# ScanNet/ScanNet

Measured on AMD Instinct MI355X. Metric: RGB-D frames/sec integrated (640x480, 4 mm voxel), higher is better.
Workload: dtype f32; 1 GPU; configs[1]: scene0000_00-scale synthetic stream (5578-frame box-room walk, 640x480 u16 depth, 4 mm voxels, 2^19 hash buckets x 10, 2^20 SDF blocks), frames 5..24 per rank, depth AND colour (a 640x480 RGB8 frame per depth frame, 921 600 B) resident in HBM; frames_per_pass=32, blocks_live_end=34141, alloc_failures=0

## Files before the change

include/scanfuse_internal.h:

```cpp
#ifndef SCANFUSE_INTERNAL_H
#define SCANFUSE_INTERNAL_H

#include "scanfuse.h"

#ifdef __cplusplus
extern "C" {
#endif

int sf_fuser_tune(sf_fuser* f, const char* key, int value);

int sf_fuser_alloc_probe_count(sf_fuser* f, uint64_t* out);

int sf_fuser_alloc_direct_count(sf_fuser* f, uint64_t* out);

int sf_fuser_mc_timing(const sf_fuser* f, double* out, int n);

int sf_zlib_inflate_gpu(const void* src, uint64_t src_bytes, uint64_t expect_bytes, int device, void* dst);
int sf_zlib_inflate_gpu_bench(const void* const* srcs, const uint64_t* src_bytes, int count, uint64_t expect_bytes, int device, int repeats, int skip, double* us_tokens, double* us_copy);

int sf_fuse_run_device_counts(uint64_t out[4]);

int sf_jpeg_decode_gpu_huffman(const uint8_t* data, uint64_t bytes, uint32_t width, uint32_t height, int device, uint8_t* dst_rgb);

int sf_fuser_profile_enable(sf_fuser* f, int on);
// ... 2 lines not shown
int sf_synth_room_device(void* d_depth, uint64_t frame_stride_bytes, uint64_t first_frame, uint64_t n, uint64_t total_frames,
                         int width, int height, int noise, float* poses_out);
int sf_synth_scan_device(void* d_depth, uint64_t frame_stride_bytes, uint64_t first_frame, uint64_t n, uint64_t total_frames,
                         int width, int height, int noise, const double room_m[3], const double origin_m[3], float* poses_out);

int sf_synth_scene_device(void* d_depth, uint64_t frame_stride_bytes, uint64_t first_frame, uint64_t n, uint64_t total_frames,
                          int width, int height, int noise, int scene, uint32_t seed, const double room_m[3], const double origin_m[3],
                          float* poses_out);
int sf_synth_clutter_boxes(const double room_m[3], uint32_t seed, float* lo_out , float* hi_out , int* n_out);

struct sf_mesh;
int sf_simplify_probe_edge(const struct sf_mesh* in, const sf_simplify_params* p, uint32_t v0, uint32_t v1, double quadric10[10], float position[3],
                           float* priority, double* scale_factor);

int sf_simplify_stage_edges(int device, uint32_t V, uint32_t F, const float* pos, const uint32_t* tri, const uint8_t* alive, const double* Q_in ,
                            const sf_simplify_params* p, double scale, uint64_t needed, int stalled, uint32_t* E_out, uint64_t* ukey, uint32_t* ucnt,
                            double* Q_out, float* pri, float* x, float* tau_out, double* scale_out );
int sf_simplify_stage_winners(int device, uint32_t V, uint32_t F, const uint32_t* tri, const uint8_t* alive, uint32_t E_in, const float* pri, float tau,
                              uint32_t round, uint8_t* pass_out, uint8_t* taken_out, uint32_t counters[3]);
int sf_simplify_stage_collapse(int device, uint32_t V, uint32_t F, float* pos, uint32_t* tri, uint8_t* alive, double* Q, uint32_t n, const uint32_t* edges,
                               uint32_t E_in, const float* x, uint8_t* vdel_out);

int sf_clean_stage_merge(int device, uint32_t V, const float* pos, float radius, uint32_t* target_out, uint32_t* launches_out, uint32_t* cells_out,
                         uint32_t* merged_out);
int sf_clean_stage_faces(int device, uint32_t V, uint32_t F, const uint32_t* tri, const uint32_t* target , uint8_t* verdict_out, uint32_t* tri_out,
                         uint32_t* degenerate_out, uint32_t* duplicate_out);
int sf_clean_stage_components(int device, uint32_t F, const uint32_t* tri, uint32_t min_faces, uint32_t* root_out, uint32_t* size_out, uint8_t* keep_out,
                              uint32_t counters[3]);
int sf_clean_stage_compact(int device, uint32_t V, uint32_t F, const float* pos, const uint8_t* col , const uint32_t* tri, uint32_t* used_out,
                           uint32_t* remap_out, float* pos_out, uint8_t* col_out, uint32_t* tri_out, uint32_t* vertices_out);
int sf_clean_probe_merge(uint32_t V, const float* pos, float radius, uint32_t* target_out);

int sf_selftest_division(int device, uint64_t* recip_mismatches, uint64_t* quot_mismatches, uint64_t* div_mismatches);

int sf_fuser_calib_tile_rmw(sf_fuser* f, int read_only, int iters, double* avg_us, uint32_t* tiles);
int sf_fuser_calib_tile_rmw_ex(sf_fuser* f, int mode, int iters, double* avg_us, uint32_t* tiles);

int sf_fuser_track_system(sf_fuser* f, const uint16_t* depth, int level, const float T[16], const float T_ref[16], const sf_track_params* t,
                          double sys[29], uint8_t* mask);

int sf_fuser_track_rgbd_system(sf_fuser* f, const uint16_t* depth, const uint8_t* rgb, int level, const float T[16], const float T_ref[16],
                               const sf_track_params* t, double sys[31], uint8_t* mask);

int sf_fuser_align_system(sf_fuser* f, const uint16_t* depth, uint64_t K, const float* poses, const int32_t* pairs, uint64_t P, const sf_align_params* a,
                          double* sys);
int sf_fuser_align_rgbd_system(sf_fuser* f, const uint16_t* depth, const uint8_t* rgb, uint64_t K, const float* poses, const int32_t* pairs, uint64_t P,
                               const sf_align_params* a, double* sys);

int sf_align_group_solve_stage(int device, uint64_t G, const int32_t* group_first, const int32_t* pair_first, const int32_t* local_pairs,
                               const uint32_t* valid_masks, const double* sys, int nsys, int min_pair_correspondences, double* xi_out, int32_t* status_out,
                               int32_t* used_out, uint32_t* conn_out, double* sums_out);

int sf_filter2d_stage_prepare(int device, const uint16_t* depth16, int dn, const uint8_t* rgb, int cn, float* depth_out, float* intensity_out);
int sf_filter2d_stage_bilateral(int device, const float* in, float sigma_d, float sigma_r, int w, int h, float* out);
int sf_filter2d_stage_resample_float(int device, const float* in, int iw, int ih, float* out, int ow, int oh);
int sf_filter2d_stage_resample_uchar(int device, const uint8_t* in, int iw, int ih, uint8_t* out, int ow, int oh);
int sf_filter2d_stage_vote(int device, const uint8_t* instance_in, const float* depth, const float* intensity, const uint8_t instance_to_idx[256],
                           const uint8_t idx_to_instance[80], int radius, int w, int h, float sigma_d, float sigma_r, float intensity_scale,
                           uint8_t* instance_out);
int sf_filter2d_stage_to_label(int device, const uint8_t* instance, const uint16_t instance_to_label[256], int n, uint16_t* label_out);
int sf_filter2d_selftest_gauss(int device, float sigma, const float* dist, const int32_t* dx, const int32_t* dy, uint64_t n, float* out_r, float* out_d);

int sf_axis_align_stage_up(const struct sf_sens* sens, uint32_t gravity_min_records, float up3[3], int32_t* source, uint64_t* no_gravity);
int sf_axis_align_stage_normals(const float* xyz, uint64_t num_vertices, const uint32_t* tris, uint64_t num_faces, int device, float* normals_out);
int sf_axis_align_stage_planes(const float* xyz, const float* normals, uint64_t num_vertices, const sf_axis_align_params* p, int device, uint32_t* index_out,
                               uint64_t* n_founded, uint32_t* ids, float* table10, uint32_t* counts, uint32_t* behind, uint64_t capacity, uint64_t* n_sorted,
// ... 31 lines not shown
```

scannet_amd/csrc/calib.hip:

```cpp
#include <hip/hip_runtime.h>

#include "common.h"
#include "fuser_internal.h"

namespace {
__global__ __launch_bounds__(256) void k_calib_rmw(uint4* __restrict__ buf, size_t n16) {
  for (size_t i = (size_t)blockIdx.x * 256 + threadIdx.x; i < n16; i += (size_t)gridDim.x * 256) {
    uint4 v = buf[i];
    v.x += 1u; v.y ^= v.x; v.z += v.y; v.w ^= v.z;
    buf[i] = v;
  }
}
__global__ __launch_bounds__(256) void k_calib_read(const uint4* __restrict__ buf, size_t n16, uint32_t* sink) {
  uint32_t acc = 0;
  for (size_t i = (size_t)blockIdx.x * 256 + threadIdx.x; i < n16; i += (size_t)gridDim.x * 256) {
    const uint4 v = buf[i];
    acc ^= v.x ^ v.y ^ v.z ^ v.w;
  }
  if (acc == 0x12345u) *sink = acc;
}
}

SF_API int sf_calib_stream(int device, uint64_t bytes, int iters) {
  SF_HIP_CHECK(hipSetDevice(device));
// ... 34 lines not shown
    const uint32_t e = 100u + (uint32_t)(x >> 58);
    n0 = __uint_as_float(((uint32_t)x & 0x807FFFFFu) | (e << 23));
    const float qf = __uint_as_float(0x3F800000u | ((uint32_t)(x >> 24) & 0x7FFFFFu));
    n1 = __uint_as_float(__float_as_uint(qf * m) + ((uint32_t)(x >> 50) & 7u) - 3u);
  }
  const v2f q = quot_rn((v2f){n0, n1}, splat(m), splat(r));
  unsigned int n = (__float_as_uint(q.x) != __float_as_uint(n0 / m)) + (__float_as_uint(q.y) != __float_as_uint(n1 / m));
  if (n) atomicAdd(bad, (unsigned long long)n);
}
__global__ __launch_bounds__(256) void k_selftest_div(unsigned long long* bad) {
  const uint64_t i = (uint64_t)blockIdx.x * 256 + threadIdx.x;
  uint64_t x = (i + 1) * 0x9E3779B97F4A7C15ull;
  x ^= x >> 29; x *= 0xBF58476D1CE4E5B9ull; x ^= x >> 32;
  uint64_t y = (x ^ 0xD6E8FEB86659FD93ull) * 0x94D049BB133111EBull;
  y ^= y >> 31;
  const uint32_t eb = 103u + (uint32_t)(x >> 58) % 41u;
  const uint32_t ea = 97u + (uint32_t)(y >> 58) % 43u;
  const float b = __uint_as_float(((uint32_t)x & 0x807FFFFFu) | (eb << 23));
  const float a0 = __uint_as_float(((uint32_t)y & 0x807FFFFFu) | (ea << 23));
  const float qf = __uint_as_float(0x3F800000u | ((uint32_t)(y >> 24) & 0x7FFFFFu));
  const float a1 = __uint_as_float(__float_as_uint(qf * b) + ((uint32_t)(x >> 50) & 7u) - 3u);
  const float qh = __uint_as_float(__float_as_uint(qf) & 0xFFFFFFFEu);
  const float a2 = __uint_as_float(__float_as_uint(fmaf(qh, b, 0x1p-24f * b)) + ((uint32_t)(y >> 50) & 7u) - 3u);
  const float a3 = __uint_as_float(__float_as_uint(a0) ^ 0x00400000u);
  const float rb = recip_rn(b);
  unsigned int n = 0;
  n += __float_as_uint(div_rn(a0, b, rb)) != __float_as_uint(a0 / b);
  n += __float_as_uint(div_rn(a1, b, rb)) != __float_as_uint(a1 / b);
  n += __float_as_uint(div_rn(a2, b, rb)) != __float_as_uint(a2 / b);
  n += __float_as_uint(div_rn(a3, b, rb)) != __float_as_uint(a3 / b);
  n += __float_as_uint(rb) != __float_as_uint(1.0f / b);
  if (n) atomicAdd(bad, (unsigned long long)n);
}
}

SF_API int sf_selftest_division(int device, uint64_t* recip_mismatches, uint64_t* quot_mismatches, uint64_t* div_mismatches) {
  if (!recip_mismatches || !quot_mismatches || !div_mismatches) return sf::fail(SF_ERR_INVALID_ARG, "NULL argument");
  SF_HIP_CHECK(hipSetDevice(device));
  unsigned long long* d = nullptr;
  SF_HIP_CHECK(hipMalloc((void**)&d, 24));
  SF_HIP_CHECK(hipMemset(d, 0, 24));
  hipLaunchKernelGGL(k_selftest_recip, dim3((1u << 23) / 256), dim3(256), 0, nullptr, d);
  hipLaunchKernelGGL(k_selftest_quot, dim3((1u << 20) / 256, 511), dim3(256), 0, nullptr, d + 1);
  hipLaunchKernelGGL(k_selftest_div, dim3((1u << 26) / 256), dim3(256), 0, nullptr, d + 2);
  unsigned long long h[3] = {0, 0, 0};
  const hipError_t e = hipMemcpy(h, d, 24, hipMemcpyDeviceToHost);
  (void)hipFree(d);
  if (e != hipSuccess) return sf::fail(SF_ERR_DEVICE, "self-test failed: %s", hipGetErrorString(e));
  *recip_mismatches = h[0];
  *quot_mismatches = h[1];
  *div_mismatches = h[2];
  return SF_OK;
}
```

scannet_amd/csrc/fuser_alloc.hip:

```cpp
#include <hip/hip_runtime.h>

#include <algorithm>
#include <climits>
#include <cmath>

#include "fuser_device.h"
#include "fuser_internal.h"

namespace {

__device__ inline int world_to_block(float w, float voxel, float rv) {
  const float q = div_rn(w, voxel, rv);
  const int vi = (int)(q >= 0.0f ? q + 0.5f : q - 0.5f);
  return vi >> 3;
}

constexpr int ALLOC_SET = 256;
constexpr int ALLOC_LIST = 512;
constexpr int ALLOC_SET_PROBES = 32;

template <int WIN_LOG2, bool MULTI>
__global__ __launch_bounds__(256) void k_alloc(const float* __restrict__ depthf_all, HashEntry* table, int32_t* heap,
                                               uint64_t* block_keys, int32_t* block_entry, uint8_t* block_flags, int32_t* counters, ParamsK P,
                                               BatchFrames B, int group_frames, BrickCache bricks) {
// ... 444 lines not shown
    const float slu = du_ * inv * (float)sgn, slv = dv_ * inv * (float)sgn;
    const float a0 = ((float)k0 + 0.5f) - oa;
    const float iu = ou_ + du_ * inv * a0 - (float)(RW_LAT / 2), iv = ov_ + dv_ * inv * a0 - (float)(RW_LAT / 2);
    const float fiu = floorf(iu), fiv = floorf(iv);
    w_axis = __builtin_amdgcn_readfirstlane(axis); w_k0 = __builtin_amdgcn_readfirstlane(k0); w_sgn = __builtin_amdgcn_readfirstlane(sgn);
    w_su = __builtin_amdgcn_readfirstlane((int)rintf(slu * 4096.0f)); w_ou = __builtin_amdgcn_readfirstlane((int)fiu);
    w_fu = __builtin_amdgcn_readfirstlane((int)((iu - fiu) * 4096.0f));
    w_sv = __builtin_amdgcn_readfirstlane((int)rintf(slv * 4096.0f)); w_ov = __builtin_amdgcn_readfirstlane((int)fiv);
    w_fv = __builtin_amdgcn_readfirstlane((int)((iv - fiv) * 4096.0f));
  };
  int n_map = max(1, j_end - j_begin);
  if (MULTI && j_end - j_begin > 1) {
    float d0[3], o0[3], d1[3], o1[3];
    centre_ray(j_begin, d0, o0);
    centre_ray(j_end - 1, d1, o1);
    const float far = P.maxd / bs;
    float D = 0.0f;
#pragma unroll
    for (int r = 0; r < 3; r++) D = fmaxf(D, fabsf((o1[r] + d1[r] * far) - (o0[r] + d0[r] * far)));
    if (D > 9.0f) n_map = max(1, (int)((float)(j_end - j_begin) * 9.0f / D));
    n_map = __builtin_amdgcn_readfirstlane(n_map);
  }
  int next_map = j_begin;
  const bool in_image = x < P.W && y < P.H;
  const float kx = ((float)x - P.mx) / P.fx, ky = ((float)y - P.my) / P.fy;
  const float rvoxel = 1.0f / P.voxel;
  float d_next;
  if (fuse_depth16 != nullptr) {
    if (blockIdx.x == 0 && blockIdx.y == 0 && threadIdx.x == 0) atomicExch(reinterpret_cast<unsigned long long*>(&counters[compact_counter]), 0ull);
    d_next = -INFINITY;
    if (in_image) {
      const uint16_t u = fuse_depth16[(size_t)(y * P.W + x)];
      float v = (float)u / P.depth_shift;
      if (u == 0 || v < P.dmin || v > P.dmax) v = -INFINITY;
      depthf_out[(size_t)(y * P.W + x)] = v;
      d_next = v;
    }
  } else {
    d_next = in_image && j_begin < j_end ? depthf_all[(size_t)j_begin * npx + (size_t)(y * P.W + x)] : -INFINITY;
  }
  __syncthreads();
  for (int j = j_begin; j < j_end; ++j) {
    const FrameK& F = B.f[j];
    const float d_cur = d_next;
    d_next = in_image && j + 1 < j_end ? depthf_all[(size_t)(j + 1) * npx + (size_t)(y * P.W + x)] : -INFINITY;
    if (j == next_map) {
      anchor(j, min(j + n_map, j_end) - 1);
      next_map = j + n_map;
      if (MULTI && j != j_begin)
        for (int i = threadIdx.x; i < RW_WORDS / 4; i += 256) s_done4[i] = make_uint4(0, 0, 0, 0);
    }

    bool active = false;
    int a_cx = 0, a_cy = 0, a_cz = 0, a_sx = 0, a_sy = 0, a_sz = 0, a_ex = 0, a_ey = 0, a_ez = 0;
    float a_tmx = INFINITY, a_tmy = INFINITY, a_tmz = INFINITY, a_tdx = INFINITY, a_tdy = INFINITY, a_tdz = INFINITY;
    if (in_image) {
      const float d = d_cur;
      if (d != -INFINITY && d < P.maxd) {
        const float t = fmaf(P.tscale, d, P.tbase);
        const float lo = min_f32(P.maxd, d - t);
        const float hi = min_f32(P.maxd, d + t);
        if (lo < hi) {
          float p0[3], p1[3];
          {
            const float ax = kx * lo, ay = ky * lo, az = lo;
#pragma unroll
            for (int r = 0; r < 3; r++) p0[r] = fmaf(F.T[4 * r], ax, fmaf(F.T[4 * r + 1], ay, fmaf(F.T[4 * r + 2], az, F.T[4 * r + 3])));
// ... 211 lines not shown
```

scannet_amd/csrc/fuser_fuse.h:

```cpp
#pragma once
#include <hip/hip_runtime.h>

#include "fuser_device.h"
#include "fuser_internal.h"

namespace {


constexpr int RTAB = 512;

struct FrameV {
  float ti[12];
  float fx, fy, mx, my, tscale, tbase;
};
__device__ inline FrameV frame_constants(const ParamsK& P, const float* __restrict__ Ti) {
  FrameV F;
#pragma unroll
  for (int k = 0; k < 12; k++) F.ti[k] = Ti[k];
  F.fx = P.fx; F.fy = P.fy; F.mx = P.mx; F.my = P.my;
  F.tscale = P.tscale; F.tbase = P.tbase;
  return F;
}

__device__ inline int cvt_i32(float x) {
  int r;
  asm("v_cvt_i32_f32 %0, %1" : "=v"(r) : "v"(x));
  return r;
}

__device__ inline uint32_t add_sat_u32(uint32_t a, uint32_t b) {
  uint32_t r;
  asm("v_add_u32_e64 %0, %1, %2 clamp" : "=v"(r) : "v"(a), "s"(b));
  return r;
}

__device__ inline int depth_weight(const ParamsK& P, float d) {
  const float z01 = (d - P.dmin) / (P.dmax - P.dmin);
  const float wf = fmaxf(((float)P.wsample * 1.5f) * (1.0f - z01), 1.0f);
  return min(cvt_i32(wf), 255);
}

template <int J0, int NJ, bool CLAMP>
__device__ inline void fuse_project(const ParamsK& P, const FrameV& FV, v2f wx, float wy, const float (&wz)[4], v2f (&pz)[NJ],
                                    uint32_t (&pix)[2 * NJ], bool (&ok)[2 * NJ]) {
  const float* Ti = FV.ti;
  const uint32_t uw = (uint32_t)P.W, uh = (uint32_t)P.H;
  v2f axy[NJ], azz[NJ / 2];
#pragma unroll
  for (int j = 0; j < NJ; j++)
    axy[j] = pk_fma((v2f){Ti[1], Ti[5]}, splat(wy), pk_fma((v2f){Ti[2], Ti[6]}, splat(wz[J0 + j]), (v2f){Ti[3], Ti[7]}));
#pragma unroll
  for (int jj = 0; jj < NJ / 2; jj++)
    azz[jj] = pk_fma(splat(Ti[9]), splat(wy), pk_fma(splat(Ti[10]), (v2f){wz[J0 + 2 * jj], wz[J0 + 2 * jj + 1]}, splat(Ti[11])));
#pragma unroll
  for (int j = 0; j < NJ; j++) {
    const v2f pcx = pk_fma(splat(Ti[0]), wx, splat(axy[j].x));
    const v2f pcy = pk_fma(splat(Ti[4]), wx, splat(axy[j].y));
    const v2f pcz = pk_fma(splat(Ti[8]), wx, splat(azz[j >> 1][j & 1]));
    const v2f rz = recip_rn(pcz);
    const v2f uf = pk_add(pk_fma(pcx * splat(FV.fx), rz, splat(FV.mx)), splat(0.5f));
    const v2f vf = pk_add(pk_fma(pcy * splat(FV.fy), rz, splat(FV.my)), splat(0.5f));
    pz[j] = pcz;
#pragma unroll
    for (int hx = 0; hx < 2; hx++) {
      const uint32_t px = (uint32_t)cvt_i32(uf[hx]), py = (uint32_t)cvt_i32(vf[hx]);
      const bool in = (pcz[hx] > 0.0f) && (px < uw) && (py < uh);
      const uint32_t p = __umul24(py, uw) + px;
      ok[2 * j + hx] = in;
      pix[2 * j + hx] = CLAMP ? (in ? p : 0u) : p;
    }
  }
}

template <int J0, int NJ>
__device__ inline void fuse_project_xr(const ParamsK& P, const FrameV& FV, const v2f (&wxp)[4], float wy, float wz, v2f (&pz)[NJ],
                                       uint32_t (&pix)[2 * NJ], bool (&ok)[2 * NJ]) {
  const float* Ti = FV.ti;
  const uint32_t uw = (uint32_t)P.W, uh = (uint32_t)P.H;
  const float ax = fmaf(Ti[1], wy, fmaf(Ti[2], wz, Ti[3]));
  const float ay = fmaf(Ti[5], wy, fmaf(Ti[6], wz, Ti[7]));
  const float az = fmaf(Ti[9], wy, fmaf(Ti[10], wz, Ti[11]));
#pragma unroll
  for (int j = 0; j < NJ; j++) {
    const v2f pcx = pk_fma(splat(Ti[0]), wxp[J0 + j], splat(ax));
    const v2f pcy = pk_fma(splat(Ti[4]), wxp[J0 + j], splat(ay));
    const v2f pcz = pk_fma(splat(Ti[8]), wxp[J0 + j], splat(az));
    const v2f rz = recip_rn(pcz);
    const v2f uf = pk_add(pk_fma(pcx * splat(FV.fx), rz, splat(FV.mx)), splat(0.5f));
    const v2f vf = pk_add(pk_fma(pcy * splat(FV.fy), rz, splat(FV.my)), splat(0.5f));
    pz[j] = pcz;
#pragma unroll
    for (int hx = 0; hx < 2; hx++) {
      const uint32_t px = (uint32_t)cvt_i32(uf[hx]), py = (uint32_t)cvt_i32(vf[hx]);
      const bool in = (pcz[hx] > 0.0f) && (px < uw) && (py < uh);
      ok[2 * j + hx] = in;
      pix[2 * j + hx] = __umul24(py, uw) + px;
    }
  }
}

template <int SIGN, int COLOR, bool TAB, int WM, int J0, int NJ, bool ROWS = true>
__device__ inline void fuse_update(const ParamsK& P, const FrameV& FV, const v2f (&rcp_m)[NJ], const float (&d)[2 * NJ], const uint32_t (&c)[2 * NJ], const v2f (&pz)[NJ],
                                   const bool (&ok)[2 * NJ], uint4 (&v)[4], uint64_t (&dirty)[4]) {
  constexpr bool WS1 = WM == 1 || WM == 2;
  const float wn = (float)P.wsample;
  const uint32_t round_mask = P.colour_round ? 0x010101u : 0u;
  const uint32_t first_mask = P.colour_first ? 0x00FFFFFFu : 0xFF000000u;
  constexpr bool wdep = WM == 3;
  const uint32_t maxd_bits = __float_as_uint(P.maxd);
  v2f q[NJ], sdfc[NJ];
  v2f wnv[NJ];
  int wni[2 * NJ];
  uint32_t ncw[2 * NJ];
  bool upd[2 * NJ];
  bool sat[2 * NJ];
  bool any_upd = false;
#pragma unroll
  for (int j = 0; j < NJ; j++) {
    const v2f dk = {d[2 * j], d[2 * j + 1]};
    v2f sdf = dk - pz[j];
    const v2f t = pk_fma(splat(FV.tscale), dk, splat(FV.tbase));
#pragma unroll
    for (int hx = 0; hx < 2; hx++) {
      upd[2 * j + hx] = ok[2 * j + hx] && (__float_as_uint(dk[hx]) < maxd_bits) && (sdf[hx] > -t[hx]);
      sdf[hx] = min_f32(sdf[hx], t[hx]);
      sat[2 * j + hx] = false;
      any_upd = any_upd || upd[2 * j + hx];
      wni[2 * j + hx] = wdep ? depth_weight(P, dk[hx]) : P.wsample;
    }
    wnv[j] = wdep ? (v2f){(float)wni[2 * j], (float)wni[2 * j + 1]} : splat(wn);
    sdfc[j] = sdf;
  }
  if (!__any((int)any_upd)) return;
  bool slow = false;
#pragma unroll
  for (int j = 0; j < NJ; j++) {
    const v2f sdf = sdfc[j];
    const uint32_t cwj[2] = {v[J0 + j].y, v[J0 + j].w};
    const v2f wo = {(float)(cwj[0] >> 24), (float)(cwj[1] >> 24)};
    const v2f old = {__uint_as_float(v[J0 + j].x), __uint_as_float(v[J0 + j].z)};
    if (SIGN > 0) {
      const v2f n = pk_fma(old, wo, WS1 ? sdf : sdf * wnv[j]);
      const v2f m = wo + wnv[j];
      if (TAB) {
        q[j] = quot_rn(n, m, rcp_m[j]);
        slow = slow || (fabsf(n.x) < 0x1p-100f) || (fabsf(n.y) < 0x1p-100f);
      } else {
        q[j] = (v2f){n.x / m.x, n.y / m.y};
      }
#pragma unroll
      for (int hx = 0; hx < 2; hx++) {
        const uint32_t cw = cwj[hx];
        const uint32_t w = cw >> 24;
        uint32_t rgb = cw;
        if (COLOR) {
          const uint32_t ck = c[2 * j + hx];
          const uint32_t avg = __builtin_amdgcn_lerp(cw, ck, round_mask);
          const bool first = COLOR == 2 ? cw < 0x01000000u : (cw & first_mask) == 0u;
          rgb = first ? ck : avg;
        }
        if (WM == 2) {
          if (COLOR) {
            ncw[2 * j + hx] = (rgb & 0x00FFFFFFu) | (add_sat_u32(cw, 0x01000000u) & 0xFF000000u);
          } else {
            uint32_t inc;
            const bool full = __builtin_add_overflow(cw, 0x01000000u, &inc);
// ... 14 lines not shown
      for (int hx = 0; hx < 2; hx++) {
        const int nw = (int)(cwj[hx] >> 24) - wni[2 * j + hx];
        if (nw <= 0) { q[j][hx] = __uint_as_float(0u); ncw[2 * j + hx] = 0u; }
        else ncw[2 * j + hx] = (cwj[hx] & 0xFFFFFFu) | ((uint32_t)nw << 24);
      }
    }
  }
  if (SIGN > 0 && TAB && __builtin_expect(__any((int)slow), 0)) {
#pragma unroll
    for (int j = 0; j < NJ; j++) {
      const v2f wo = {(float)(v[J0 + j].y >> 24), (float)(v[J0 + j].w >> 24)};
      const v2f old = {__uint_as_float(v[J0 + j].x), __uint_as_float(v[J0 + j].z)};
      const v2f n = pk_fma(old, wo, sdfc[j] * wnv[j]);
      const v2f m = wo + wnv[j];
      q[j] = (v2f){n.x / m.x, n.y / m.y};
    }
  }
#pragma unroll
  for (int j = 0; j < NJ; j++) {
    v[J0 + j].x = upd[2 * j] ? __float_as_uint(q[j].x) : v[J0 + j].x;
    v[J0 + j].y = (upd[2 * j] && !sat[2 * j]) ? ncw[2 * j] : v[J0 + j].y;
    v[J0 + j].z = upd[2 * j + 1] ? __float_as_uint(q[j].y) : v[J0 + j].z;
    v[J0 + j].w = (upd[2 * j + 1] && !sat[2 * j + 1]) ? ncw[2 * j + 1] : v[J0 + j].w;
    if (ROWS) dirty[J0 + j] |= __ballot(upd[2 * j] || upd[2 * j + 1]);
  }
  if (!ROWS) dirty[0] = ~0ull;
}


__device__ inline __amdgpu_buffer_rsrc_t image_rsrc(const void* base, uint32_t bytes) {
  return __builtin_amdgcn_make_buffer_rsrc(const_cast<void*>(base), 0, (int)bytes, 0x00020000);
}

template <int SIGN, int COLOR, bool TAB, int WM, int J0, int NJ, bool ROWS, bool XR = false>
__device__ inline void fuse_rows(const ParamsK& P, const float* __restrict__ Ti, const float* __restrict__ depthf,
                                 const uint2* __restrict__ texel, const float* rtab, v2f wx, float wy, const float (&wz)[4], const v2f (&wxp)[4],
                                 uint4 (&v)[4], uint64_t (&dirty)[4]) {
  v2f pz[NJ], rcp_m[NJ];
  float d[2 * NJ];
  uint32_t c[2 * NJ];
  bool ok[2 * NJ];
  uint32_t pix[2 * NJ];
  if (TAB) {
#pragma unroll
    for (int j = 0; j < NJ; j++) {
      const uint32_t ws = (WM == 1 || WM == 2) ? 1u : (uint32_t)P.wsample;
      rcp_m[j] = (v2f){rtab[(v[J0 + j].y >> 24) + ws], rtab[(v[J0 + j].w >> 24) + ws]};
    }
  }
  const FrameV FV = frame_constants(P, Ti);
  if (XR) fuse_project_xr<J0, NJ>(P, FV, wxp, wy, wz[0], pz, pix, ok);
  else fuse_project<J0, NJ, false>(P, FV, wx, wy, wz, pz, pix, ok);
  const uint32_t img_bytes = (uint32_t)(P.W * P.H) * 4u;
  if (COLOR) {
    typedef uint32_t u32x2 __attribute__((ext_vector_type(2)));
    const __amdgpu_buffer_rsrc_t rt = image_rsrc(texel, 2u * img_bytes);
#pragma unroll
    for (int k = 0; k < 2 * NJ; k++) {
      const u32x2 t = __builtin_amdgcn_raw_buffer_load_b64(rt, pix[k] << 3, 0, 0);
      d[k] = __uint_as_float(t.x);
      c[k] = t.y;
    }
  } else {
    const __amdgpu_buffer_rsrc_t rd = image_rsrc(depthf, img_bytes);
#pragma unroll
    for (int k = 0; k < 2 * NJ; k++) d[k] = __uint_as_float(__builtin_amdgcn_raw_buffer_load_b32(rd, pix[k] << 2, 0, 0));
  }
  fuse_update<SIGN, COLOR, TAB, WM, J0, NJ, ROWS>(P, FV, rcp_m, d, c, pz, ok, v, dirty);
}

}
```

scannet_amd/csrc/fuser_internal.h:

```cpp
#pragma once
#include <hip/hip_runtime.h>

#include <utility>
#include <vector>

#include "common.h"

constexpr uint64_t KEY_EMPTY = ~0ull;
constexpr uint64_t KEY_TOMB = ~0ull - 1ull;
constexpr int MAX_DDA_ITERS = 1024;
constexpr int MAX_PROBES = 4096;
constexpr int MAX_BATCH = 32;
constexpr int DEFAULT_BATCH = 32;

struct HashEntry {
  uint64_t key;
  int32_t ptr;
  uint32_t birth;
};
static_assert(sizeof(HashEntry) == 16, "hash entry is 16 bytes");

struct ParamsK {
  int W, H;
  float fx, fy, mx, my;
// ... 133 lines not shown
    if (t == 0ull) t = tag;
  }
  if (t == tag) atomicOr(e + 1, 1ull << brick_bit(bx, by, bz));
}

#endif

__device__ inline int hash_lookup(const HashEntry* __restrict__ table, const ParamsK& P, int x, int y, int z) {
  const uint64_t key = pack_key(x, y, z);
  uint32_t slot = hash_home(P, x, y, z);
  for (int probe = 0; probe < MAX_PROBES; ++probe) {
    const uint64_t k = table[slot].key;
    if (k == key) return table[slot].ptr;
    if (k == KEY_EMPTY) return -1;
    slot++;
    if (slot == P.total_slots) slot = 0;
  }
  return -1;
}

#ifdef __HIPCC__
struct v2f {
  float x, y;
  __device__ float& operator[](int i) { return i ? y : x; }
  __device__ const float& operator[](int i) const { return i ? y : x; }
};
__device__ inline v2f operator+(v2f a, v2f b) { return v2f{a.x + b.x, a.y + b.y}; }
__device__ inline v2f operator-(v2f a, v2f b) { return v2f{a.x - b.x, a.y - b.y}; }
__device__ inline v2f operator*(v2f a, v2f b) { return v2f{a.x * b.x, a.y * b.y}; }
__device__ inline v2f operator-(v2f a) { return v2f{-a.x, -a.y}; }
__device__ inline v2f pk_fma(v2f a, v2f b, v2f c) { return v2f{__builtin_fmaf(a.x, b.x, c.x), __builtin_fmaf(a.y, b.y, c.y)}; }
__device__ inline v2f splat(float x) { return v2f{x, x}; }
__device__ inline v2f pk_add(v2f a, v2f b) { return a + b; }
__device__ inline v2f recip_rn(v2f b) {
  v2f r = {__builtin_amdgcn_rcpf(b.x), __builtin_amdgcn_rcpf(b.y)};
  const v2f one = splat(1.0f);
  r = pk_fma(pk_fma(-b, r, one), r, r);
  return pk_fma(pk_fma(-b, r, one), r, r);
}
__device__ inline float recip_rn(float b) {
  float r = __builtin_amdgcn_rcpf(b);
  r = fmaf(fmaf(-b, r, 1.0f), r, r);
  return fmaf(fmaf(-b, r, 1.0f), r, r);
}
__device__ inline float div_rn(float a, float b, float y) {
  const float q0 = a * y;
  const float q1 = fmaf(fmaf(-b, q0, a), y, q0);
  return fmaf(fmaf(-b, q1, a), y, q1);
}
__device__ inline v2f quot_rn(v2f n, v2f m, v2f r) {
  const v2f q0 = n * r;
  return pk_fma(pk_fma(-m, q0, n), r, q0);
}
#endif

struct sf_fuser {
  sf_params p;
  ParamsK pk;
  int in_W = 0, in_H = 0;
  size_t in_px = 0;
  int device = 0;
  hipStream_t stream = nullptr;
  hipStream_t front = nullptr;
  hipStream_t front_lo = nullptr;
  hipStream_t last_front = nullptr;
  hipEvent_t ev_front_switch = nullptr;
  int front_prio = -1;
  bool front_lo_lowest = true;
  hipEvent_t ev_compact[2] = {nullptr, nullptr};
  hipEvent_t ev_fused[2] = {nullptr, nullptr};
  hipEvent_t ev_input = nullptr;
  int slot = 0;
  bool serial_tail = false;
// ... 83 lines not shown
```

scannet_amd/csrc/fuser_prepass.hip:

```cpp
#include <hip/hip_runtime.h>

#include <algorithm>
#include <cmath>

#include "fuser_internal.h"
#include "jpeg_idct.h"

namespace {

struct YccPicture {
  int ncomp, sx[3], sy[3], cw[3], ch[3], bw[3];
  const uint8_t* plane[3];
  __device__ YccPicture(const SfJpegLayout* __restrict__ L, const uint8_t* planes) {
    const int W = L->width, H = L->height;
    ncomp = L->ncomp;
    const uint8_t* q = planes;
    for (int c = 0; c < 3; c++) {
      const int cc = c < ncomp ? c : 0;
      sx[c] = L->hmax > L->h[cc] ? 2 : 1; sy[c] = L->vmax > L->v[cc] ? 2 : 1;
      cw[c] = (W + sx[c] - 1) >> (sx[c] - 1); ch[c] = (H * L->v[cc] + L->vmax - 1) >> (L->vmax - 1);
      bw[c] = L->bw[cc];
      plane[c] = q;
      if (c < ncomp) q += (size_t)L->bw[cc] * L->bh[cc];
    }
// ... 17 lines not shown
__global__ __launch_bounds__(256) void k_prepass(BatchIn in, float* __restrict__ depthf_all, uint2* __restrict__ texel_all, int n,
                                                 float shift, float dmin, float dmax, int32_t* counters, int compact_counter, ParamsK P,
                                                 const float* __restrict__ ray_kx, const float* __restrict__ ray_ky) {
  const int j = blockIdx.y;
  const uint16_t* __restrict__ depth = in.depth[j];
  const uint8_t* __restrict__ rgb = in.rgb[j];
  float* __restrict__ depthf = depthf_all + (size_t)j * n;
  uint2* __restrict__ texel = texel_all + (size_t)j * n;
  const int i0 = (blockIdx.x * 256 + threadIdx.x) * 8;
  if (blockIdx.x == 0 && j == 0 && threadIdx.x == 0) {
    atomicExch(reinterpret_cast<unsigned long long*>(&counters[compact_counter]), 0ull);
  }
  const bool ycc = rgb != nullptr && in.lay[j] != nullptr;
  if (i0 >= n && !ycc) return;
  uint16_t u[8];
  if (P.inW > 0) {
    for (int k = 0; k < 8; k++) {
      const int i = i0 + k;
      if (i >= n) { u[k] = 0; continue; }
      const unsigned xi = (unsigned)((float)(i % P.W) * P.rsx + 0.5f), yi = (unsigned)((float)(i / P.W) * P.rsy + 0.5f);
      u[k] = (xi < (unsigned)P.inW && yi < (unsigned)P.inH) ? depth[(size_t)yi * P.inW + xi] : (uint16_t)0;
    }
  } else if (i0 + 8 <= n) {
    const uint4 raw = *reinterpret_cast<const uint4*>(depth + i0);
    u[0] = raw.x & 0xFFFF; u[1] = raw.x >> 16; u[2] = raw.y & 0xFFFF; u[3] = raw.y >> 16;
    u[4] = raw.z & 0xFFFF; u[5] = raw.z >> 16; u[6] = raw.w & 0xFFFF; u[7] = raw.w >> 16;
  } else {
    for (int k = 0; k < 8; k++) u[k] = (i0 + k < n) ? depth[i0 + k] : (uint16_t)0;
  }
  float d[8];
#pragma unroll
  for (int k = 0; k < 8; k++) {
    float v = (float)u[k] / shift;
    if (u[k] == 0 || v < dmin || v > dmax) v = -INFINITY;
    d[k] = v;
  }
  if (i0 + 8 <= n) {
    *reinterpret_cast<float4*>(depthf + i0) = make_float4(d[0], d[1], d[2], d[3]);
    *reinterpret_cast<float4*>(depthf + i0 + 4) = make_float4(d[4], d[5], d[6], d[7]);
  } else {
    for (int k = 0; k < 8 && i0 + k < n; k++) depthf[i0 + k] = d[k];
  }
  if (ycc) {
    __shared__ float s_d[2048];
#pragma unroll
    for (int k = 0; k < 8; k++) s_d[threadIdx.x * 8 + k] = d[k];
    __syncthreads();
    const YccPicture pic(reinterpret_cast<const SfJpegLayout*>(in.lay[j]), rgb);
    const int wg0 = blockIdx.x * 2048;
#pragma unroll 2
    for (int k = 0; k < 8; k++) {
      const int p = wg0 + k * 256 + (int)threadIdx.x;
      if (p >= n) break;
      const int y = p / P.W, x = p - y * P.W;
      uint32_t c = 0u;
      if (P.cW == 0) c = pic.pixel(x, y);
      else {
        const float u = fmaf(ray_kx[x], P.cfx, P.cmx) + 0.5f;
        const float v = fmaf(ray_ky[y], P.cfy, P.cmy) + 0.5f;
        if (u >= 0.0f && u < (float)P.cW && v >= 0.0f && v < (float)P.cH) c = pic.pixel((int)u, (int)v);
      }
      texel[p] = make_uint2(__float_as_uint(s_d[k * 256 + (int)threadIdx.x]), c);
    }
  } else if (rgb) {
    if (P.cW == 0) {
      if (i0 + 8 <= n && ((uintptr_t)rgb & 7) == 0) {
        const uint2* q = reinterpret_cast<const uint2*>(rgb + 3 * (size_t)i0);
// ... 50 lines not shown
```

scannet_amd/csrc/fuser_reintegrate.hip:

```cpp
#include <hip/hip_runtime.h>

#include <algorithm>
#include <atomic>
#include <chrono>
#include <cmath>
#include <cstring>
#include <thread>
#include <vector>

#include "fuser_device.h"
#include "fuser_fuse.h"
#include "fuser_internal.h"

namespace {

constexpr int REINT_WAVES = 5;

template <int COLOR, bool TAB, int WM, bool XR>
__global__ __launch_bounds__(256, REINT_WAVES) void k_reintegrate(uint4* __restrict__ voxels, const uint64_t* __restrict__ block_keys,
                                                                  const int32_t* __restrict__ compact, const uint32_t* __restrict__ cmask,
                                                                  const float* __restrict__ depthf_all, const uint2* __restrict__ texel_all,
                                                                  int32_t* counters, int32_t* host_mirror, int compact_counter, int xcd_walk, ParamsK P,
                                                                  BatchTi B, ReintSlots R) {
  __shared__ float s_rtab[RTAB];
// ... 17 lines not shown
  const int chunk = xcd_walk ? (wg_total + 7) >> 3 : wg_total;
  const int lanes = xcd_walk ? 8 : 1;
  const int sub = xcd_walk ? (int)(blockIdx.x & 7) : 0;
  const int per_sub = max(1, (int)gridDim.x / lanes);
  for (int loc = xcd_walk ? (int)(blockIdx.x >> 3) : (int)blockIdx.x; loc < chunk; loc += per_sub) {
    const int i = ((sub * chunk + loc) << 2) + wave;
    if (i >= n) continue;
    const int slot = compact[i];
    uint32_t slots = (uint32_t)__builtin_amdgcn_readfirstlane((int)cmask[i]);
    int bx, by, bz;
    unpack_key(block_keys[slot], bx, by, bz);
    uint4* vb = voxels + (size_t)slot * 256;
    uint4 v[4];
#pragma unroll
    for (int j = 0; j < 4; j++) v[j] = vb[XR ? lane * 4 + j : j * 64 + lane];
    const v2f wx = {(float)(8 * bx + lx) * P.voxel, (float)(8 * bx + lx + 1) * P.voxel};
    const float wy = (float)(8 * by + ly) * P.voxel;
    float wz[4];
    v2f wxp[4];
#pragma unroll
    for (int j = 0; j < 4; j++) {
      wz[j] = (float)(8 * bz + (XR ? 0 : 2 * j) + lzb) * P.voxel;
      wxp[j] = v2f{(float)(8 * bx + 2 * j) * P.voxel, (float)(8 * bx + 2 * j + 1) * P.voxel};
    }
    uint64_t dirty[4] = {0ull, 0ull, 0ull, 0ull};
    while (slots != 0u) {
      const int q = __builtin_ctz(slots);
      slots &= slots - 1u;
      const float* Ti = B.Ti[q];
      const size_t im = (size_t)R.img[q];
      const float* __restrict__ depthf = depthf_all + im * npx;
      const uint2* __restrict__ texel = texel_all + im * npx;
      if ((R.neg >> q) & 1u) fuse_rows<-1, 0, false, WMN, 0, 4, false, XR>(P, Ti, depthf, texel, s_rtab, wx, wy, wz, wxp, v, dirty);
      else fuse_rows<1, COLOR, TAB, WM, 0, 4, false, XR>(P, Ti, depthf, texel, s_rtab, wx, wy, wz, wxp, v, dirty);
    }
    if (dirty[0] != 0ull) {
#pragma unroll
      for (int j = 0; j < 4; j++) vb[XR ? lane * 4 + j : j * 64 + lane] = v[j];
    }
  }
}

struct ReintegrateLaunch {
  const sf_fuser* f;
  int sl;
  const BatchTi& bt;
  const ReintSlots& rs;
  hipStream_t s;

  template <int COLOR, bool TAB, int WM, bool XR>
  void run() const {
    const int grid = sf_list_grid(f, *f->host_mirror);
    hipLaunchKernelGGL((k_reintegrate<COLOR, TAB, WM, XR>), dim3(grid), dim3(256), 0, s, f->voxels, f->block_keys, f->compact2[sl], f->cmask2[sl],
                       f->depthf2[sl], f->color2[sl], f->counters, f->host_mirror, sf_compact_counter(sl), f->xcd_walk ? 1 : 0, f->pk, bt, rs);
  }
  template <bool TAB, int WM>
  void colour(bool col) const {
    if (col) run<1, TAB, WM, false>();
    else run<0, TAB, WM, false>();
  }
};

}

void sf_launch_reintegrate(const sf_fuser* f, int sl, bool col, const BatchTi& bt, const ReintSlots& rs, hipStream_t s) {
  const ReintegrateLaunch L{f, sl, bt, rs, s};
  const bool ws1 = f->p.weight_sample == 1 && f->p.weight_mode == 0;
// ... 158 lines not shown
```

Measured before the change: 35210 frames/s.

## Streamline fuse inner loop: one-step reciprocal, hoisted depth cap, predicated SDF update

Replaces the two-Newton-step reciprocal with a single refinement step and adds a self-test that counts mismatches against IEEE division. The max-depth check moves from the per-voxel update into the depth prepass, and a wave-uniform all-in-front test skips per-element z>0 checks. A new predicated update path for the common TAB/WM==2 case computes the weighted SDF average with an FMA correction and inline-asm writes, falling back to true division only when the numerator is tiny. The intent is fewer VALU instructions per voxel-frame in the fuse kernel. The cost is possible last-ulp differences from the one-step reciprocal, and the reintegration path opts out of the predicated update.

```diff
diff --git a/include/scanfuse_internal.h b/include/scanfuse_internal.h
--- a/include/scanfuse_internal.h
+++ b/include/scanfuse_internal.h
@@ -58,6 +58,7 @@
 int sf_clean_probe_merge(uint32_t V, const float* pos, float radius, uint32_t* target_out);
 
 int sf_selftest_division(int device, uint64_t* recip_mismatches, uint64_t* quot_mismatches, uint64_t* div_mismatches);
+int sf_selftest_recip_one_step(int device, uint64_t* mismatches, uint32_t* patterns_out, uint32_t capacity, int* shipped);
 
 int sf_fuser_calib_tile_rmw(sf_fuser* f, int read_only, int iters, double* avg_us, uint32_t* tiles);
 int sf_fuser_calib_tile_rmw_ex(sf_fuser* f, int mode, int iters, double* avg_us, uint32_t* tiles);
diff --git a/scannet_amd/csrc/calib.hip b/scannet_amd/csrc/calib.hip
--- a/scannet_amd/csrc/calib.hip
+++ b/scannet_amd/csrc/calib.hip
@@ -90,6 +90,44 @@
   n += __float_as_uint(rb) != __float_as_uint(1.0f / b);
   if (n) atomicAdd(bad, (unsigned long long)n);
 }
+__global__ __launch_bounds__(256) void k_selftest_recip_one_step(unsigned long long* bad, uint32_t* first, uint32_t capacity) {
+  const uint32_t base = (blockIdx.x * 256u + threadIdx.x) << 4;
+  for (uint32_t k = 0; k < 16u; k++) {
+    const uint32_t bits = base | k;
+    const float b = __uint_as_float(bits);
+    const uint32_t ref = __float_as_uint(1.0f / b);
+    const uint32_t eb = (bits >> 23) & 0xFFu, er = (ref >> 23) & 0xFFu;
+    if (eb == 0u || eb == 255u || er == 0u || er == 255u) continue;
+    if (__float_as_uint(recip_one_step(b)) != ref) {
+      const unsigned long long slot = atomicAdd(bad, 1ull);
+      if (slot < (unsigned long long)capacity) first[slot] = bits;
+    }
+  }
+}
+}
+
+SF_API int sf_selftest_recip_one_step(int device, uint64_t* mismatches, uint32_t* patterns_out, uint32_t capacity, int* shipped) {
+  if (!mismatches || (capacity > 0 && !patterns_out)) return sf::fail(SF_ERR_INVALID_ARG, "NULL argument");
+  SF_HIP_CHECK(hipSetDevice(device));
+  unsigned long long* d = nullptr;
+  uint32_t* p = nullptr;
+  SF_HIP_CHECK(hipMalloc((void**)&d, 8));
+  if (hipMalloc((void**)&p, 4 * (size_t)(capacity ? capacity : 1)) != hipSuccess) { (void)hipFree(d); return sf::fail(SF_ERR_DEVICE, "self-test: hipMalloc failed"); }
+  hipError_t e = hipMemset(d, 0, 8);
+  if (e == hipSuccess) e = hipMemset(p, 0, 4 * (size_t)(capacity ? capacity : 1));
+  if (e == hipSuccess) {
+    hipLaunchKernelGGL(k_selftest_recip_one_step, dim3(1u << 20), dim3(256), 0, nullptr, d, p, capacity);
+    e = hipGetLastError();
+  }
+  unsigned long long h = 0;
+  if (e == hipSuccess) e = hipMemcpy(&h, d, 8, hipMemcpyDeviceToHost);
+  if (e == hipSuccess && capacity > 0) e = hipMemcpy(patterns_out, p, 4 * (size_t)capacity, hipMemcpyDeviceToHost);
+  (void)hipFree(d);
+  (void)hipFree(p);
+  if (e != hipSuccess) return sf::fail(SF_ERR_DEVICE, "self-test failed: %s", hipGetErrorString(e));
+  *mismatches = h;
+  if (shipped) *shipped = RECIP_ONE_STEP ? 1 : 0;
+  return SF_OK;
 }
 
 SF_API int sf_selftest_division(int device, uint64_t* recip_mismatches, uint64_t* quot_mismatches, uint64_t* div_mismatches) {
diff --git a/scannet_amd/csrc/fuser_alloc.hip b/scannet_amd/csrc/fuser_alloc.hip
--- a/scannet_amd/csrc/fuser_alloc.hip
+++ b/scannet_amd/csrc/fuser_alloc.hip
@@ -500,7 +500,7 @@
     if (in_image) {
       const uint16_t u = fuse_depth16[(size_t)(y * P.W + x)];
       float v = (float)u / P.depth_shift;
-      if (u == 0 || v < P.dmin || v > P.dmax) v = -INFINITY;
+      if (u == 0 || v < P.dmin || v > P.dmax || !(v < P.maxd)) v = -INFINITY;
       depthf_out[(size_t)(y * P.W + x)] = v;
       d_next = v;
     }
diff --git a/scannet_amd/csrc/fuser_fuse.h b/scannet_amd/csrc/fuser_fuse.h
--- a/scannet_amd/csrc/fuser_fuse.h
+++ b/scannet_amd/csrc/fuser_fuse.h
@@ -32,6 +32,13 @@
   uint32_t r;
   asm("v_add_u32_e64 %0, %1, %2 clamp" : "=v"(r) : "v"(a), "s"(b));
   return r;
+}
+
+__device__ inline void write_fma(uint32_t& dst, float a, float b, float c) {
+  asm volatile("v_fma_f32 %0, %1, %2, %3" : "+v"(dst) : "v"(a), "v"(b), "v"(c));
+}
+__device__ inline void write_bfi(uint32_t& dst, uint32_t mask, uint32_t a, uint32_t b) {
+  asm volatile("v_bfi_b32 %0, %1, %2, %3" : "+v"(dst) : "s"(mask), "v"(a), "v"(b));
 }
 
 __device__ inline int depth_weight(const ParamsK& P, float d) {
@@ -81,25 +88,32 @@
   const float ay = fmaf(Ti[5], wy, fmaf(Ti[6], wz, Ti[7]));
   const float az = fmaf(Ti[9], wy, fmaf(Ti[10], wz, Ti[11]));
 #pragma unroll
+  for (int j = 0; j < NJ; j++) pz[j] = pk_fma(splat(Ti[8]), wxp[J0 + j], splat(az));
+  const bool front = (__ballot(pz[0].x > 0.0f) & __ballot(pz[NJ - 1].y > 0.0f)) == __ballot(1);
+  bool zpos[2 * NJ];
+#pragma unroll
+  for (int k = 0; k < 2 * NJ; k++) zpos[k] = true;
+  if (__builtin_expect(!front, 0)) {
+#pragma unroll
+    for (int k = 0; k < 2 * NJ; k++) zpos[k] = pz[k >> 1][k & 1] > 0.0f;
+  }
+#pragma unroll
   for (int j = 0; j < NJ; j++) {
     const v2f pcx = pk_fma(splat(Ti[0]), wxp[J0 + j], splat(ax));
     const v2f pcy = pk_fma(splat(Ti[4]), wxp[J0 + j], splat(ay));
-    const v2f pcz = pk_fma(splat(Ti[8]), wxp[J0 + j], splat(az));
-    const v2f rz = recip_rn(pcz);
+    const v2f rz = recip_rn(pz[j]);
     const v2f uf = pk_add(pk_fma(pcx * splat(FV.fx), rz, splat(FV.mx)), splat(0.5f));
     const v2f vf = pk_add(pk_fma(pcy * splat(FV.fy), rz, splat(FV.my)), splat(0.5f));
-    pz[j] = pcz;
 #pragma unroll
     for (int hx = 0; hx < 2; hx++) {
       const uint32_t px = (uint32_t)cvt_i32(uf[hx]), py = (uint32_t)cvt_i32(vf[hx]);
-      const bool in = (pcz[hx] > 0.0f) && (px < uw) && (py < uh);
-      ok[2 * j + hx] = in;
+      ok[2 * j + hx] = zpos[2 * j + hx] && (px < uw) && (py < uh);
       pix[2 * j + hx] = __umul24(py, uw) + px;
     }
   }
 }
 
-template <int SIGN, int COLOR, bool TAB, int WM, int J0, int NJ, bool ROWS = true>
+template <int SIGN, int COLOR, bool TAB, int WM, int J0, int NJ, bool ROWS = true, bool PRED = true>
 __device__ inline void fuse_update(const ParamsK& P, const FrameV& FV, const v2f (&rcp_m)[NJ], const float (&d)[2 * NJ], const uint32_t (&c)[2 * NJ], const v2f (&pz)[NJ],
                                    const bool (&ok)[2 * NJ], uint4 (&v)[4], uint64_t (&dirty)[4]) {
   constexpr bool WS1 = WM == 1 || WM == 2;
@@ -107,7 +121,6 @@
   const uint32_t round_mask = P.colour_round ? 0x010101u : 0u;
   const uint32_t first_mask = P.colour_first ? 0x00FFFFFFu : 0xFF000000u;
   constexpr bool wdep = WM == 3;
-  const uint32_t maxd_bits = __float_as_uint(P.maxd);
   v2f q[NJ], sdfc[NJ];
   v2f wnv[NJ];
   int wni[2 * NJ];
@@ -122,7 +135,7 @@
     const v2f t = pk_fma(splat(FV.tscale), dk, splat(FV.tbase));
 #pragma unroll
     for (int hx = 0; hx < 2; hx++) {
-      upd[2 * j + hx] = ok[2 * j + hx] && (__float_as_uint(dk[hx]) < maxd_bits) && (sdf[hx] > -t[hx]);
+      upd[2 * j + hx] = ok[2 * j + hx] && (sdf[hx] > -t[hx]);
       sdf[hx] = min_f32(sdf[hx], t[hx]);
       sat[2 * j + hx] = false;
       any_upd = any_upd || upd[2 * j + hx];
@@ -132,6 +145,60 @@
     sdfc[j] = sdf;
   }
   if (!__any((int)any_upd)) return;
+  if constexpr (PRED && SIGN > 0 && TAB && WM == 2) {
+    v2f q0[NJ], e[NJ];
+    bool tiny = false;
+#pragma unroll
+    for (int j = 0; j < NJ; j++) {
+      const v2f wo = {(float)(v[J0 + j].y >> 24), (float)(v[J0 + j].w >> 24)};
+      const v2f old = {__uint_as_float(v[J0 + j].x), __uint_as_float(v[J0 + j].z)};
+      const v2f n = pk_fma(old, wo, sdfc[j]);
+      const v2f m = wo + splat(wn);
+      q0[j] = n * rcp_m[j];
+      e[j] = pk_fma(-m, q0[j], n);
+      tiny = tiny || (fabsf(n.x) < 0x1p-100f) || (fabsf(n.y) < 0x1p-100f);
+    }
+    if (__builtin_expect(__any((int)tiny) != 0, 0)) {
+#pragma unroll
+      for (int j = 0; j < NJ; j++) {
+        const v2f wo = {(float)(v[J0 + j].y >> 24), (float)(v[J0 + j].w >> 24)};
+        const v2f old = {__uint_as_float(v[J0 + j].x), __uint_as_float(v[J0 + j].z)};
+        const v2f n = pk_fma(old, wo, sdfc[j]);
+        const v2f m = wo + splat(wn);
+        q0[j] = (v2f){n.x / m.x, n.y / m.y};
+        e[j] = splat(-0.0f);
+      }
+    }
+#pragma unroll
+    for (int j = 0; j < NJ; j++) {
+#pragma unroll
+      for (int hx = 0; hx < 2; hx++) {
+        const int k = 2 * j + hx;
+        uint32_t& sdf_word = hx ? v[J0 + j].z : v[J0 + j].x;
+        uint32_t& cw_word = hx ? v[J0 + j].w : v[J0 + j].y;
+        const uint32_t cw = cw_word;
+        uint32_t rgb = cw, wsum = 0u;
+        bool keep = false;
+        if (COLOR) {
+          const uint32_t ck = c[k];
+          const uint32_t avg = __builtin_amdgcn_lerp(cw, ck, round_mask);
+          const bool first = COLOR == 2 ? cw < 0x01000000u : (cw & first_mask) == 0u;
+          rgb = first ? ck : avg;
+          wsum = add_sat_u32(cw, 0x01000000u);
+        } else {
+          keep = __builtin_add_overflow(cw, 0x01000000u, &wsum);
+        }
+        if (upd[k]) {
+          write_fma(sdf_word, e[j][hx], rcp_m[j][hx], q0[j][hx]);
+          if (COLOR) write_bfi(cw_word, 0x00FFFFFFu, rgb, wsum);
+        }
+        if (!COLOR) cw_word = (upd[k] && !keep) ? wsum : cw_word;
+      }
+      if (ROWS) dirty[J0 + j] |= __ballot(upd[2 * j] || upd[2 * j + 1]);
+    }
+    if (!ROWS) dirty[0] = ~0ull;
+    return;
+  }
   bool slow = false;
 #pragma unroll
   for (int j = 0; j < NJ; j++) {
@@ -212,7 +279,7 @@
   return __builtin_amdgcn_make_buffer_rsrc(const_cast<void*>(base), 0, (int)bytes, 0x00020000);
 }
 
-template <int SIGN, int COLOR, bool TAB, int WM, int J0, int NJ, bool ROWS, bool XR = false>
+template <int SIGN, int COLOR, bool TAB, int WM, int J0, int NJ, bool ROWS, bool XR = false, bool PRED = true>
 __device__ inline void fuse_rows(const ParamsK& P, const float* __restrict__ Ti, const float* __restrict__ depthf,
                                  const uint2* __restrict__ texel, const float* rtab, v2f wx, float wy, const float (&wz)[4], const v2f (&wxp)[4],
                                  uint4 (&v)[4], uint64_t (&dirty)[4]) {
@@ -246,7 +313,7 @@
 #pragma unroll
     for (int k = 0; k < 2 * NJ; k++) d[k] = __uint_as_float(__builtin_amdgcn_raw_buffer_load_b32(rd, pix[k] << 2, 0, 0));
   }
-  fuse_update<SIGN, COLOR, TAB, WM, J0, NJ, ROWS>(P, FV, rcp_m, d, c, pz, ok, v, dirty);
-}
-
-}
+  fuse_update<SIGN, COLOR, TAB, WM, J0, NJ, ROWS, PRED>(P, FV, rcp_m, d, c, pz, ok, v, dirty);
+}
+
+}
diff --git a/scannet_amd/csrc/fuser_internal.h b/scannet_amd/csrc/fuser_internal.h
--- a/scannet_amd/csrc/fuser_internal.h
+++ b/scannet_amd/csrc/fuser_internal.h
@@ -189,13 +189,20 @@
 __device__ inline v2f pk_fma(v2f a, v2f b, v2f c) { return v2f{__builtin_fmaf(a.x, b.x, c.x), __builtin_fmaf(a.y, b.y, c.y)}; }
 __device__ inline v2f splat(float x) { return v2f{x, x}; }
 __device__ inline v2f pk_add(v2f a, v2f b) { return a + b; }
+__device__ inline float recip_one_step(float b) {
+  const float r = __builtin_amdgcn_rcpf(b);
+  return fmaf(fmaf(-b, r, 1.0f), r, r);
+}
+constexpr bool RECIP_ONE_STEP = true;
 __device__ inline v2f recip_rn(v2f b) {
+  if (RECIP_ONE_STEP) return v2f{recip_one_step(b.x), recip_one_step(b.y)};
   v2f r = {__builtin_amdgcn_rcpf(b.x), __builtin_amdgcn_rcpf(b.y)};
   const v2f one = splat(1.0f);
   r = pk_fma(pk_fma(-b, r, one), r, r);
   return pk_fma(pk_fma(-b, r, one), r, r);
 }
 __device__ inline float recip_rn(float b) {
+  if (RECIP_ONE_STEP) return recip_one_step(b);
   float r = __builtin_amdgcn_rcpf(b);
   r = fmaf(fmaf(-b, r, 1.0f), r, r);
   return fmaf(fmaf(-b, r, 1.0f), r, r);
diff --git a/scannet_amd/csrc/fuser_prepass.hip b/scannet_amd/csrc/fuser_prepass.hip
--- a/scannet_amd/csrc/fuser_prepass.hip
+++ b/scannet_amd/csrc/fuser_prepass.hip
@@ -73,7 +73,7 @@
 #pragma unroll
   for (int k = 0; k < 8; k++) {
     float v = (float)u[k] / shift;
-    if (u[k] == 0 || v < dmin || v > dmax) v = -INFINITY;
+    if (u[k] == 0 || v < dmin || v > dmax || !(v < P.maxd)) v = -INFINITY;
     d[k] = v;
   }
   if (i0 + 8 <= n) {
diff --git a/scannet_amd/csrc/fuser_reintegrate.hip b/scannet_amd/csrc/fuser_reintegrate.hip
--- a/scannet_amd/csrc/fuser_reintegrate.hip
+++ b/scannet_amd/csrc/fuser_reintegrate.hip
@@ -73,7 +73,7 @@
       const float* __restrict__ depthf = depthf_all + im * npx;
       const uint2* __restrict__ texel = texel_all + im * npx;
       if ((R.neg >> q) & 1u) fuse_rows<-1, 0, false, WMN, 0, 4, false, XR>(P, Ti, depthf, texel, s_rtab, wx, wy, wz, wxp, v, dirty);
-      else fuse_rows<1, COLOR, TAB, WM, 0, 4, false, XR>(P, Ti, depthf, texel, s_rtab, wx, wy, wz, wxp, v, dirty);
+      else fuse_rows<1, COLOR, TAB, WM, 0, 4, false, XR, false>(P, Ti, depthf, texel, s_rtab, wx, wy, wz, wxp, v, dirty);
     }
     if (dirty[0] != 0ull) {
 #pragma unroll
```

Measured after the change: 36700 frames/s (median of 6 runs). 1.04x the previous value.
